# YoungSean/UnseenObjectsWithMeanShift

Measured on AMD Instinct MI355X. Metric: images/sec @640x480 RGB-D, 100 queries, 9 decoder layers; % MFMA roofline, higher is better.
Workload: dtype f32; 1 GPU; configs[1]: batch 8 of 640x480 per GPU, ResNet-50 features -> MSDeformAttn pixel decoder -> 9-layer decoder, 100 q ->~; global_batch=8, per_gpu_batch=8, launch=hipgraph x4: 4 batches of 8 in flight, one graph + stream each, batches_in_flight=4, parallelism=dp1, GPU_MAX_HW_QUEUES=4, visible_gpus=1, rank0_numa=pinned

## Files before the change

### include/msm_hip.h

```cpp
#ifndef MSM_HIP_H
#define MSM_HIP_H

#include <stdint.h>

#ifdef __cplusplus
extern "C" {
#endif

#define MSM_OK 0
#define MSM_E_INVALID (-1)
#define MSM_E_LAUNCH (-2)
#define MSM_E_WORKSPACE (-3)

const char* msm_last_error_string(void);
#define MSM_ABI_VERSION 24
int msm_abi_version(void);

#define MSM_OPT_AUTO (-1)
enum {
    MSM_OPT_MASK_NC = 0,
    MSM_OPT_MASKB_TARGET,
    MSM_OPT_GEMM_TILE,
    MSM_OPT_GEMM_SHALLOW,
    MSM_OPT_ATTN_TARGET,
    MSM_OPT_ATTN_KERNEL,
    MSM_OPT_ATTN_QK_MAX,
    MSM_OPT_ATTN_QKCFG,
    MSM_OPT_CONVIN_NT,
    MSM_OPT_POST_GENERIC,
    MSM_OPT_ENC_NO_COOP,
    MSM_OPT_MSDA_GENERIC,
    MSM_OPT_MS_CHUNK,
    MSM_OPT_MS_NO_PERSISTENT,
    MSM_OPT_ATTN_FUSED_KV,
    MSM_OPT_KV_PIPE,
    MSM_OPT_MASK_KERNEL,
    MSM_OPT_MS_SPLIT_KERNEL,
    MSM_OPT_CONV3_WIDE,
    MSM_OPT_DEC_TILE32,
    MSM_OPT_COUNT
};
int msm_set_option(int key, int value);
int msm_get_option(int key);

int msm_gemm_f32(const float* A, const float* A2, const float* W, const float* bias, float* C,
                 int M, int N, int K, int batch,
                 int64_t a_sm, int64_t a_sk, int64_t a_sb, int64_t a2_sb, int64_t w_sb,
                 int64_t c_sm, int64_t c_sn, int64_t c_sb, int64_t c_ss,
                 int a_mode, int conv_h, int conv_w, int conv_c,
                 int bias_mode, int act, int split_k, void* stream);

int msm_layernorm_f32(const float* x, const float* parts, int n_parts, int64_t part_stride,
                      const float* bias, const float* g1, const float* b1, int l2norm,
                      const float* g2, const float* b2, float* y, float* y2,
                      int rows, int E, float eps, void* stream);

int msm_groupnorm_stats_f32(const float* x, double* stats, int stats_cleared, int B, int HW, int C, void* stream);
int msm_groupnorm_apply_f32(const float* x, const double* stats, const float* gamma, const float* beta,
                            const float* up, int uh, int uw, int64_t up_batch_stride, float* y,
                            int B, int H, int W, int C, int groups, float eps, int relu, void* stream);

int msm_groupnorm_apply_split(const float* x, const double* stats, const float* gamma, const float* beta,
                              const float* up, int uh, int uw, int64_t up_batch_stride, uint16_t* planes,
                              int B, int H, int W, int C, int groups, float eps, int relu, void* stream);

int msm_groupnorm_apply_f16(const float* x, const double* stats, const float* gamma, const float* beta,
                            const float* up, int uh, int uw, int64_t up_batch_stride, void* y_f16,
                            int B, int H, int W, int C, int groups, float eps, int relu, void* stream);
// ... 34 lines not shown
int64_t msm_hypersphere_attn_workspace(int B, int Lq, int S, int heads);
int msm_hypersphere_attn_fwd(const float* q, const float* k, const float* v,
                             const uint8_t* masked, const int32_t* row_any, float* out,
                             int B, int Lq, int S, int heads,
                             int64_t ldq, int64_t q_sb, int64_t ldk, int64_t k_sb,
                             int64_t ldv, int64_t v_sb, float kappa,
                             float* workspace, int64_t workspace_elems, void* stream);
int msm_hypersphere_attn_lp_fwd(const float* q, const void* k, const void* v, int kv_format,
                                const uint8_t* masked, const int32_t* row_any, float* out,
                                int B, int Lq, int S, int heads,
                                int64_t ldq, int64_t q_sb, int64_t ldk, int64_t k_sb,
                                int64_t ldv, int64_t v_sb, float kappa,
                                float* workspace, int64_t workspace_elems, void* stream);

int msm_nchw_to_tokens_f16(const float* in, void* out, int B, int C, int HW, void* stream);
int msm_attn_pack_kv_weights(const float* w, void* packed, int heads, void* stream);
int msm_mask_conv3x3_folded(const void* x_f16, const float* F, int64_t ldf, int64_t f_sb, void* mask_bits, int32_t* row_any, int row_any_cleared,
                            float* logits, int B, int Q, int H, int W, void* stream);
int64_t msm_attn_mask_bits_bytes(int B, int Lq, int S);
int msm_attn_pack_mask_bits(const uint8_t* masked, void* bits, int B, int Lq, int S, void* stream);
int msm_hypersphere_attn_fused_kv_fwd(const float* q, const void* x_f16, const void* w_packed, const float* rowcol, const float* col_v_t,
                                      int score_format, const void* mask_bits, const int32_t* row_any, float* out,
                                      int B, int Lq, int H, int W, int heads, int64_t ldq, int64_t q_sb, float kappa,
                                      float* workspace, int64_t workspace_elems, void* stream);

int msm_msdeform_attn_fwd(const float* value, const int64_t* spatial_shapes,
                          const int64_t* level_start_index, const float* sampling_loc,
                          const float* attn_weight, float* out,
                          int B, int S, int M, int D, int L, int Lq, int P, void* stream);

int msm_msdeform_attn_bwd(const float* value, const int64_t* spatial_shapes,
                          const int64_t* level_start_index, const float* sampling_loc,
                          const float* attn_weight, const float* grad_output,
                          float* grad_value, float* grad_sampling_loc, float* grad_attn_weight,
                          int B, int S, int M, int D, int L, int Lq, int P, void* stream);
int msm_msdeform_attn_fwd_f64(const double* value, const int64_t* spatial_shapes,
                              const int64_t* level_start_index, const double* sampling_loc,
                              const double* attn_weight, double* out,
                              int B, int S, int M, int D, int L, int Lq, int P, void* stream);
int msm_msdeform_attn_bwd_f64(const double* value, const int64_t* spatial_shapes,
                              const int64_t* level_start_index, const double* sampling_loc,
                              const double* attn_weight, const double* grad_output,
                              double* grad_value, double* grad_sampling_loc, double* grad_attn_weight,
                              int B, int S, int M, int D, int L, int Lq, int P, void* stream);

int msm_msdeform_attn_enc_fwd(const float* value, const int64_t* spatial_shapes,
                              const int64_t* level_start_index, const float* proj, float* out,
                              int B, int S, int M, int D, int L, int P, void* stream);

int msm_value_to_head_major_f32(const float* value, float* value_hm, int B, int S, int M, int D, void* stream);
int msm_msdeform_attn_enc_hm_fwd(const float* value_hm, const int64_t* spatial_shapes,
                                 const int64_t* level_start_index, const float* proj, float* out,
                                 int B, int S, int M, int D, int L, int P, void* stream);

int msm_msda_pack_proj(const float* w , const float* bias, float* wpack, float* bpack,
                       int M, int L, int P, void* stream);
int msm_msdeform_attn_enc_fused_fwd(const float* value_hm, const int64_t* spatial_shapes, const int64_t* level_start_index,
                                    const float* src, const float* pos, const float* wpack, const float* bpack, float* out,
                                    int B, int S, int M, int D, int L, int P, void* stream);

int64_t msm_encoder_block_stream_floats(int d_ffn, int proj_width);
int msm_encoder_block_fwd(const float* attn, const float* src, const float* wstream, const float* small,
                          const float* pos, float* src_out, float* value_out, float* proj_out,
                          int M, int S, int d_ffn, int proj_width, int value_heads, float eps, void* stream);

int msm_kv_project_f32(const float* x, const float* w, const float* cmat, float* out,
                       int B, int C, int HW, int N, int x_tokens, int64_t x_batch_stride, int cmat_width, void* stream);
int msm_kv_project_multi_f32(int n_jobs, const float* const* x, const float* const* w, const float* const* cmat,
                             float* const* out, const int32_t* HW, const int32_t* x_tokens, const int64_t* x_batch_stride,
                             const int32_t* cmat_width, int B, int C, int N, void* stream);
int msm_kv_project_multi_bf16(int n_jobs, const float* const* x, const float* const* w, const float* const* cmat,
                              uint16_t* const* out, const int32_t* HW, const int32_t* x_tokens, const int64_t* x_batch_stride,
                              const int32_t* cmat_width, int B, int C, int N, int half_format, void* stream);
int msm_kv_project_multi_split(int n_jobs, const float* const* x, const float* const* w, const float* const* cmat,
                               float* const* out, const int32_t* HW, const int32_t* x_tokens, const int64_t* x_batch_stride,
                               const int32_t* cmat_width, int B, int C, int N, void* stream);

int msm_tokens_proj_nchw_f32(const float* x, const float* w, const float* bias, const double* gn_stats,
                             const float* gn_gamma, const float* gn_beta, int groups, float eps, int relu, float* out,
                             int B, int C, int HW, int N, void* stream);

int msm_dec_pack_weight(const float* w, float* packed, int N, int K, void* stream);
int msm_dec_post_cross(const float* attn_out, const float* res, const float* query_pos,
                       const float* wo, const float* bo, const float* ln_g, const float* ln_b,
                       const float* w_in, const float* b_in,
                       float* x_out, float* qk_out, float* v_out,
                       int rows, int Q, int E, float eps, void* stream);
int msm_dec_post_self(const float* attn_out, const float* res,
                      const float* wo, const float* bo, const float* ln_g, const float* ln_b,
                      const float* w1, const float* b1, const float* w2, int F,
                      float* x_out, float* parts, int n_parts, int rows, int E, float eps, void* stream);
int msm_dec_heads(const float* x, const float* parts, int n_parts, const float* bias,
                  const float* ln_g, const float* ln_b, int l2norm,
                  const float* dec_g, const float* dec_b,
                  const float* m0w, const float* m0b, const float* m1w, const float* m1b,
                  const float* m2w, const float* m2b,
                  const float* wq, const float* bq, const float* query_pos,
                  float* out, float* d_out, float* e_out, float* q_out, int32_t* row_any_zero,
                  int rows, int Q, int E, float eps, void* stream);

int msm_dec_pack_weight_bf16(const float* w, uint16_t* packed, int N, int K, void* stream);
int msm_dec_post_cross_bf16(const float* attn_out, const float* res, const float* query_pos,
                            const uint16_t* wo, const float* bo, const float* ln_g, const float* ln_b,
                            const uint16_t* w_in, const float* b_in,
                            float* x_out, float* qk_out, float* v_out,
                            int rows, int Q, int E, float eps, void* stream);
// ... 213 lines not shown
```

### unseenobjectswithmeanshift_amd/_lib.py

```python
import ctypes
import os
import re

_HERE = os.path.dirname(os.path.abspath(__file__))
LIB_PATH = os.path.join(_HERE, "libmsm_hip.so")
HEADER_PATH = os.path.join(os.path.dirname(_HERE), "include", "msm_hip.h")

_lib = None
ABI_VERSION = 24

c_f = ctypes.c_void_p
c_p = ctypes.c_void_p
c_i = ctypes.c_int
c_l = ctypes.c_int64
c_fl = ctypes.c_float

_SIGNATURES = {
    "msm_abi_version": (c_i, []),
    "msm_last_error_string": (ctypes.c_char_p, []),
    "msm_set_option": (c_i, [c_i, c_i]),
    "msm_get_option": (c_i, [c_i]),
    "msm_gemm_f32": (c_i, [c_f, c_f, c_f, c_f, c_f, c_i, c_i, c_i, c_i,
                           c_l, c_l, c_l, c_l, c_l, c_l, c_l, c_l, c_l,
                           c_i, c_i, c_i, c_i, c_i, c_i, c_i, c_p]),
    "msm_layernorm_f32": (c_i, [c_f, c_f, c_i, c_l, c_f, c_f, c_f, c_i, c_f, c_f, c_f, c_f, c_i, c_i, c_fl, c_p]),
    "msm_groupnorm_stats_f32": (c_i, [c_f, c_p, c_i, c_i, c_i, c_i, c_p]),
    "msm_groupnorm_apply_f32": (c_i, [c_f, c_p, c_f, c_f, c_f, c_i, c_i, c_l, c_f, c_i, c_i, c_i, c_i, c_i, c_fl, c_i, c_p]),
    "msm_groupnorm_apply_split": (c_i, [c_f, c_p, c_f, c_f, c_f, c_i, c_i, c_l, c_f, c_i, c_i, c_i, c_i, c_i, c_fl, c_i, c_p]),
    "msm_groupnorm_apply_f16": (c_i, [c_f, c_p, c_f, c_f, c_f, c_i, c_i, c_l, c_p, c_i, c_i, c_i, c_i, c_i, c_fl, c_i, c_p]),
    "msm_groupnorm_apply_nchw_f32": (c_i, [c_f, c_p, c_f, c_f, c_f, c_i, c_i, c_i, c_i, c_fl, c_i, c_p]),
    "msm_pos_embed_sine": (c_i, [c_f, c_i, c_i, c_i, c_l, c_l, c_f, c_fl, c_fl, c_p]),
    "msm_transpose_f32": (c_i, [c_f, c_f, c_i, c_i, c_i, c_p]),
    "msm_l2_normalize_nchw_f32": (c_i, [c_f, c_f, c_i, c_i, c_i, c_fl, c_p]),
    "msm_msda_locations": (c_i, [c_f, c_f, c_f, c_p, c_f, c_f, c_l, c_i, c_i, c_i, c_p]),
    "msm_mask_logits_fwd": (c_i, [c_f, c_f, c_f, c_p, c_p, c_i, c_i, c_i, c_i, c_i, c_i, c_i, c_i, c_l, c_f, c_l, c_p]),
    "msm_pool_mask_taps": (c_i, [c_f, c_i, c_i, c_i, c_i, c_p, c_p, c_p, c_p, c_l, c_p]),
    "msm_attn_mask_pooled": (c_i, [c_f, c_l, c_f, c_l, c_f, c_p, c_p, c_i, c_i, c_i, c_i, c_i, c_p]),
    "msm_pack_mask_features_bf16": (c_i, [c_f, c_p, c_i, c_i, c_i, c_p]),
    "msm_pack_mask_features_f16": (c_i, [c_f, c_p, c_i, c_i, c_i, c_p]),
    "msm_mask_logits_bf16_fwd": (c_i, [c_f, c_p, c_f, c_p, c_p, c_i, c_i, c_i, c_i, c_i, c_i, c_i, c_i, c_l, c_f, c_l, c_p]),
    "msm_pack_mask_features_split": (c_i, [c_f, c_p, c_i, c_i, c_i, c_p]),
    "msm_mask_logits_split_fwd": (c_i, [c_f, c_p, c_f, c_p, c_p, c_i, c_i, c_i, c_i, c_i, c_i, c_i, c_i, c_l, c_f, c_l, c_p]),
    "msm_hypersphere_attn_workspace": (c_l, [c_i, c_i, c_i, c_i]),
    "msm_hypersphere_attn_fwd": (c_i, [c_f, c_f, c_f, c_p, c_p, c_f, c_i, c_i, c_i, c_i,
                                       c_l, c_l, c_l, c_l, c_l, c_l, c_fl, c_f, c_l, c_p]),
    "msm_hypersphere_attn_lp_fwd": (c_i, [c_f, c_p, c_p, c_i, c_p, c_p, c_f, c_i, c_i, c_i, c_i,
                                          c_l, c_l, c_l, c_l, c_l, c_l, c_fl, c_f, c_l, c_p]),
    "msm_hypersphere_attn_bwd_workspace": (c_l, [c_i, c_i, c_i]),
    "msm_hypersphere_attn_bwd": (c_i, [c_f, c_f, c_f, c_p, c_p, c_f, c_f, c_f, c_f, c_i, c_i, c_i, c_i,
                                       c_l, c_l, c_l, c_l, c_l, c_l, c_fl, c_f, c_l, c_p]),
    "msm_msdeform_attn_fwd": (c_i, [c_f, c_p, c_p, c_f, c_f, c_f, c_i, c_i, c_i, c_i, c_i, c_i, c_i, c_p]),
    "msm_msdeform_attn_bwd": (c_i, [c_f, c_p, c_p, c_f, c_f, c_f, c_f, c_f, c_f, c_i, c_i, c_i, c_i, c_i, c_i, c_i, c_p]),
    "msm_msdeform_attn_fwd_f64": (c_i, [c_f, c_p, c_p, c_f, c_f, c_f, c_i, c_i, c_i, c_i, c_i, c_i, c_i, c_p]),
    "msm_msdeform_attn_bwd_f64": (c_i, [c_f, c_p, c_p, c_f, c_f, c_f, c_f, c_f, c_f, c_i, c_i, c_i, c_i, c_i, c_i, c_i, c_p]),
    "msm_msdeform_attn_enc_fwd": (c_i, [c_f, c_p, c_p, c_f, c_f, c_i, c_i, c_i, c_i, c_i, c_i, c_p]),
    "msm_encoder_block_stream_floats": (c_l, [c_i, c_i]),
    "msm_value_to_head_major_f32": (c_i, [c_f, c_f, c_i, c_i, c_i, c_i, c_p]),
    "msm_msdeform_attn_enc_hm_fwd": (c_i, [c_f, c_p, c_p, c_f, c_f, c_i, c_i, c_i, c_i, c_i, c_i, c_p]),
    "msm_msda_pack_proj": (c_i, [c_f, c_f, c_f, c_f, c_i, c_i, c_i, c_p]),
    "msm_msdeform_attn_enc_fused_fwd": (c_i, [c_f, c_p, c_p, c_f, c_f, c_f, c_f, c_f, c_i, c_i, c_i, c_i, c_i, c_i, c_p]),
    "msm_encoder_block_fwd": (c_i, [c_f, c_f, c_f, c_f, c_f, c_f, c_f, c_f, c_i, c_i, c_i, c_i, c_i, c_fl, c_p]),
    "msm_encoder_block_split_stream_bytes": (c_l, [c_i, c_i]),
    "msm_encoder_block_split_fwd": (c_i, [c_f, c_f, c_p, c_f, c_f, c_f, c_f, c_f, c_i, c_i, c_i, c_i, c_i, c_fl, c_p]),
    "msm_encoder_block_lp_stream_bytes": (c_l, [c_i, c_i]),
    "msm_encoder_block_lp_fwd": (c_i, [c_f, c_f, c_p, c_f, c_f, c_f, c_f, c_f, c_i, c_i, c_i, c_i, c_i, c_fl, c_p]),
    "msm_encoder_block_hm_stream_bytes": (c_l, [c_i, c_i]),
    "msm_encoder_block_hm_small_floats": (c_i, [c_i]),
    "msm_encoder_block_hm_fwd": (c_i, [c_p, c_f, c_p, c_f, c_f, c_f, c_p, c_p, c_i, c_i, c_i, c_fl, c_i, c_p]),
    "msm_msdeform_attn_enc_lp_fwd": (c_i, [c_p, c_p, c_p, c_p, c_p, c_i, c_i, c_i, c_i, c_i, c_i, c_p]),
    "msm_msdeform_attn_enc_lp_fused_fwd": (c_i, [c_p, c_p, c_p, c_f, c_f, c_p, c_f, c_p, c_i, c_i, c_i, c_i, c_i, c_i, c_p]),
    "msm_f32_to_f16": (c_i, [c_f, c_p, c_l, c_p]),
    "msm_bias_act_nhwc": (c_i, [c_p, c_p, c_p, c_i, c_l, c_i, c_i, c_p]),
    "msm_nhwc_to_nchw_f32": (c_i, [c_p, c_f, c_i, c_i, c_i, c_i, c_p]),
    "msm_ucn_embedding_tail": (c_i, [c_f, c_f, c_f, c_i, c_i, c_i, c_i, c_i, c_i, c_fl, c_p]),
    "msm_f32_to_f16_rows": (c_i, [c_f, c_p, c_i, c_l, c_l, c_p]),
    "msm_kv_project_f32": (c_i, [c_f, c_f, c_f, c_f, c_i, c_i, c_i, c_i, c_i, c_l, c_i, c_p]),
    "msm_kv_project_multi_f32": (c_i, [c_i, c_p, c_p, c_p, c_p, c_p, c_p, c_p, c_p, c_i, c_i, c_i, c_p]),
    "msm_kv_project_multi_bf16": (c_i, [c_i, c_p, c_p, c_p, c_p, c_p, c_p, c_p, c_p, c_i, c_i, c_i, c_i, c_p]),
    "msm_kv_project_multi_split": (c_i, [c_i, c_p, c_p, c_p, c_p, c_p, c_p, c_p, c_p, c_i, c_i, c_i, c_p]),
    "msm_tokens_proj_nchw_f32": (c_i, [c_f, c_f, c_f, c_p, c_f, c_f, c_i, c_fl, c_i, c_f, c_i, c_i, c_i, c_i, c_p]),
    "msm_dec_pack_weight": (c_i, [c_f, c_f, c_i, c_i, c_p]),
    "msm_dec_post_cross": (c_i, [c_f] * 12 + [c_i, c_i, c_i, c_fl, c_p]),
    "msm_dec_post_self": (c_i, [c_f] * 9 + [c_i, c_f, c_f, c_i, c_i, c_i, c_fl, c_p]),
    "msm_dec_heads": (c_i, [c_f, c_f, c_i, c_f, c_f, c_f, c_i] + [c_f] * 15 + [c_p, c_i, c_i, c_i, c_fl, c_p]),
    "msm_dec_pack_weight_bf16": (c_i, [c_f, c_p, c_i, c_i, c_p]),
    "msm_dec_post_cross_bf16": (c_i, [c_f, c_f, c_f, c_p, c_f, c_f, c_f, c_p, c_f, c_f, c_f, c_f] + [c_i, c_i, c_i, c_fl, c_p]),
    "msm_dec_post_self_bf16": (c_i, [c_f, c_f, c_p, c_f, c_f, c_f, c_p, c_f, c_p] + [c_i, c_f, c_f, c_i, c_i, c_i, c_fl, c_p]),
    "msm_dec_heads_bf16": (c_i, [c_f, c_f, c_i, c_f, c_f, c_f, c_i, c_f, c_f, c_p, c_f, c_p, c_f, c_p, c_f, c_p, c_f, c_f] + [c_f] * 4 +
                           [c_p, c_i, c_i, c_i, c_fl, c_p]),
    "msm_nchw_to_tokens_f16": (c_i, [c_f, c_p, c_i, c_i, c_i, c_p]),
    "msm_mask_conv3x3_folded": (c_i, [c_p, c_f, c_l, c_l, c_p, c_p, c_i, c_f, c_i, c_i, c_i, c_i, c_p]),
    "msm_attn_pack_kv_weights": (c_i, [c_f, c_p, c_i, c_p]),
    "msm_attn_mask_bits_bytes": (c_l, [c_i, c_i, c_i]),
    "msm_attn_pack_mask_bits": (c_i, [c_p, c_p, c_i, c_i, c_i, c_p]),
    "msm_hypersphere_attn_fused_kv_fwd": (c_i, [c_f, c_p, c_p, c_f, c_f, c_i, c_p, c_p, c_f, c_i, c_i, c_i, c_i, c_i, c_l, c_l, c_fl, c_f, c_l, c_p]),
    "msm_dec_pack_weight_f16": (c_i, [c_f, c_p, c_i, c_i, c_p]),
    "msm_dec_post_cross_f16": (c_i, [c_f, c_f, c_f, c_p, c_f, c_f, c_f, c_p, c_f, c_f, c_f, c_f] + [c_i, c_i, c_i, c_fl, c_p]),
    "msm_dec_post_self_f16": (c_i, [c_f, c_f, c_p, c_f, c_f, c_f, c_p, c_f, c_p] + [c_i, c_f, c_f, c_i, c_i, c_i, c_fl, c_p]),
    "msm_dec_heads_f16": (c_i, [c_f, c_f, c_i, c_f, c_f, c_f, c_i, c_f, c_f, c_p, c_f, c_p, c_f, c_p, c_f, c_p, c_f, c_f] + [c_f] * 4 +
                          [c_p, c_i, c_i, c_i, c_fl, c_p]),
    "msm_dec_heads_mask": (c_i, [c_f, c_f, c_i, c_f, c_f, c_f, c_i, c_f, c_f, c_p, c_f, c_p, c_f, c_p, c_f, c_p, c_f, c_f] + [c_f] * 4 +
                           [c_f, c_i, c_i, c_p, c_p, c_i, c_i, c_i, c_i, c_fl, c_p]),
    "msm_dec_pack_weight_bf16x2": (c_i, [c_f, c_p, c_i, c_i, c_p]),
    "msm_dec_post_cross_bf16x2": (c_i, [c_f, c_f, c_f, c_p, c_f, c_f, c_f, c_p, c_f, c_f, c_f, c_f] + [c_i, c_i, c_i, c_fl, c_p]),
    "msm_dec_post_self_bf16x2": (c_i, [c_f, c_f, c_p, c_f, c_f, c_f, c_p, c_f, c_p] + [c_i, c_f, c_f, c_i, c_i, c_i, c_fl, c_p]),
    "msm_dec_heads_bf16x2": (c_i, [c_f, c_f, c_i, c_f, c_f, c_f, c_i, c_f, c_f, c_p, c_f, c_p, c_f, c_p, c_f, c_p, c_f, c_f] + [c_f] * 4 +
                             [c_p, c_i, c_i, c_i, c_fl, c_p]),
    "msm_l2_prefetch": (c_i, [c_p, c_p, c_i, c_p]),
    "msm_dec_set_prefetch": (c_i, [c_p, c_p, c_i]),
    "msm_ms_seed_workspace": (c_l, [c_i]),
    "msm_ms_select_seeds": (c_i, [c_f, c_i, c_i, c_i, c_l, c_f, c_p, c_f, c_l, c_i, c_p]),
# ... 148 lines not shown
```

### unseenobjectswithmeanshift_amd/csrc/msda.hip

```cpp
#include <stdlib.h>

#include "common.h"

namespace msm {

constexpr int MAXL = 8;

template <int V>
struct Vec {
    float e[V];
};
template <int V>
__device__ __forceinline__ Vec<V> ldv(const float* p) {
    Vec<V> r;
    if constexpr (V == 4) {
        const float4 t = *reinterpret_cast<const float4*>(p);
        r.e[0] = t.x; r.e[1] = t.y; r.e[2] = t.z; r.e[3] = t.w;
    } else {
#pragma unroll
        for (int i = 0; i < V; ++i) r.e[i] = p[i];
    }
    return r;
}

// ... 322 lines not shown
                const int i = i0 + j;
                wt[j] = wb[j] = 0.f;
                vt[j] = vbm[j] = make_float4(0.f, 0.f, 0.f, 0.f);
                if (i < LP) {
                    int W = Ws[0], H = Hs[0], s0 = 0;
#pragma unroll
                    for (int l = 1; l < MAXL; ++l)
                        if (l < L && i >= l * P) { W = Ws[l]; H = Hs[l]; s0 = st[l]; }
                    const float w_im = quad_bcast(px[i >> 2], i & 3);
                    const float h_im = quad_bcast(py[i >> 2], i & 3);
                    const float wgt = quad_bcast(pw[i >> 2], i & 3) * rden;
                    const float hf = floorf(h_im), wf = floorf(w_im);
                    const int h_low = (int)hf, xw = (int)wf + cx;
                    const float lh = h_im - hf, lw = w_im - wf;
                    const float wxw = (unsigned)xw < (unsigned)W ? (cx ? lw : 1.f - lw) * wgt : 0.f;
                    wt[j] = (unsigned)h_low < (unsigned)H ? (1.f - lh) * wxw : 0.f;
                    wb[j] = (unsigned)(h_low + 1) < (unsigned)H ? lh * wxw : 0.f;
                    const int xc = clamp0(xw, W - 1);
                    const int yt = clamp0(h_low, H - 1), yb = clamp0(h_low + 1, H - 1);
                    const unsigned col = vlane + (unsigned)(s0 + xc) * (unsigned)(D * 4);
                    vt[j] = ldv4(vrsrc, col + __umul24((unsigned)yt, (unsigned)(W * D * 4)));
                    vbm[j] = ldv4(vrsrc, col + __umul24((unsigned)yb, (unsigned)(W * D * 4)));
                }
            }
#pragma unroll
            for (int j = 0; j < GP; ++j) {
                acc.x += wt[j] * vt[j].x + wb[j] * vbm[j].x;
                acc.y += wt[j] * vt[j].y + wb[j] * vbm[j].y;
                acc.z += wt[j] * vt[j].z + wb[j] * vbm[j].z;
                acc.w += wt[j] * vt[j].w + wb[j] * vbm[j].w;
            }
        }
    }
    acc.x += __int_as_float(__builtin_amdgcn_mov_dpp(__float_as_int(acc.x), 0x4E, 0xf, 0xf, true));
    acc.y += __int_as_float(__builtin_amdgcn_mov_dpp(__float_as_int(acc.y), 0x4E, 0xf, 0xf, true));
    acc.z += __int_as_float(__builtin_amdgcn_mov_dpp(__float_as_int(acc.z), 0x4E, 0xf, 0xf, true));
    acc.w += __int_as_float(__builtin_amdgcn_mov_dpp(__float_as_int(acc.w), 0x4E, 0xf, 0xf, true));
    if (live && cx == 0) *reinterpret_cast<float4*>(out + (((int64_t)b * S + qi) * M + m) * D + d4 * 4) = acc;
}

struct LevelRcp {
    float rw[4], rh[4];
};
__device__ __forceinline__ float div_by(float x, float W, float rW) {
    const float q = x * rW;
    return fmaf(fmaf(-q, W, x), rW, q);
}
__device__ __forceinline__ float exp_neg(float x) { return __builtin_amdgcn_exp2f(x * 1.4426950408889634f); }
__device__ __forceinline__ float rcp_nr(float x) {
    const float r = __builtin_amdgcn_rcpf(x);
    return fmaf(fmaf(-x, r, 1.0f), r, r);
}

template <int LC, int PC>
__global__ __launch_bounds__(256) void msda_enc_hm8_rec_kernel(const float* __restrict__ value, const int64_t* __restrict__ shapes,
                                                               const int64_t* __restrict__ lstart, const float* __restrict__ proj,
                                                               float* __restrict__ out, int B, int S, int M) {
    constexpr int D = 8, LP = LC * PC, SLOTS = LP / 4;
    static_assert(PC == 4 && LP % 4 == 0 && LP <= 16, "a lane owns one point of every level: PC == 4");
    constexpr int QSTRIDE = LP * 2 + 1;
    __shared__ float4 recs[4 * 16 * QSTRIDE];
    const int b = blockIdx.x % B;
    const int blk = blockIdx.x / B;
    const int tid = threadIdx.x, lane = tid & 63;
    const int wave = __builtin_amdgcn_readfirstlane(tid >> 6);
    const int g = tid & 3, cx = g >> 1, d4 = g & 1;
    const int m = blk % M;
    const int q_raw = (blk / M) * 64 + (tid >> 2);
    const bool live = q_raw < S;
    const int qi = live ? q_raw : 0;

    int Hs[LC], Ws[LC], st[LC];
#pragma unroll
    for (int l = 0; l < LC; ++l) {
        Hs[l] = (int)shapes[2 * l];
        Ws[l] = (int)shapes[2 * l + 1];
        st[l] = (int)lstart[l];
    }
    LevelRcp lr;
#pragma unroll
    for (int l = 0; l < LC; ++l) {
        lr.rw[l] = rcp_nr((float)Ws[l]);
        lr.rh[l] = rcp_nr((float)Hs[l]);
    }
    const float* pr = proj + ((int64_t)b * S + qi) * (M * LP * 3);
    const float* offp = pr + (int64_t)m * LP * 2;
    const float* lgp = pr + (int64_t)M * LP * 2 + (int64_t)m * LP;
    int qW = Ws[0], qH = Hs[0], qs = 0;
    float qrw = lr.rw[0], qrh = lr.rh[0];
#pragma unroll
    for (int l = 1; l < LC; ++l)
        if (qi >= st[l]) { qW = Ws[l]; qH = Hs[l]; qs = st[l]; qrw = lr.rw[l]; qrh = lr.rh[l]; }
    const int local = qi - qs;
    const int ry = (int)(((float)local + 0.5f) * qrw), rx = local - ry * qW;
    const float ref_x = div_by((float)rx + 0.5f, (float)qW, qrw);
    const float ref_y = div_by((float)ry + 0.5f, (float)qH, qrh);

    float px[SLOTS], py[SLOTS], pw[SLOTS];
    float mx = -INFINITY;
#pragma unroll
    for (int slot = 0; slot < SLOTS; ++slot) {
        const int i = slot * 4 + g;
        const float2 off = *reinterpret_cast<const float2*>(offp + 2 * i);
        const float lg = lgp[i];
        const float lx = ref_x + div_by(off.x, (float)Ws[slot], lr.rw[slot]);
        const float ly = ref_y + div_by(off.y, (float)Hs[slot], lr.rh[slot]);
        px[slot] = lx * (float)Ws[slot] - 0.5f;
        py[slot] = ly * (float)Hs[slot] - 0.5f;
        pw[slot] = lg;
        mx = fmaxf(mx, lg);
    }
    mx = quad_max(mx);
    float den = 0.f;
#pragma unroll
    for (int slot = 0; slot < SLOTS; ++slot) {
        pw[slot] = exp_neg(pw[slot] - mx);
        den += pw[slot];
    }
    const float rden = rcp_nr(quad_sum(den));

    float4* qrec = recs + (wave * 16 + (lane >> 2)) * QSTRIDE;
#pragma unroll
    for (int slot = 0; slot < SLOTS; ++slot) {
        const int W = Ws[slot], H = Hs[slot], s0 = st[slot];
        const float w_im = px[slot], h_im = py[slot];
        const float wgt = pw[slot] * rden;
        const float hf = floorf(h_im), wf = floorf(w_im);
        const int h_low = (int)hf, w_low = (int)wf;
        const float lh = h_im - hf, lw = w_im - wf;
        const float wx0 = (unsigned)w_low < (unsigned)W ? (1.f - lw) * wgt : 0.f;
        const float wx1 = (unsigned)(w_low + 1) < (unsigned)W ? lw * wgt : 0.f;
        const bool okt = (unsigned)h_low < (unsigned)H, okb = (unsigned)(h_low + 1) < (unsigned)H;
        const unsigned rowt = __umul24((unsigned)clamp0(h_low, H - 1), (unsigned)(W * D * 4));
        const unsigned rowb = __umul24((unsigned)clamp0(h_low + 1, H - 1), (unsigned)(W * D * 4));
        const unsigned c0 = (unsigned)(s0 + clamp0(w_low, W - 1)) * (unsigned)(D * 4);
        const unsigned c1 = (unsigned)(s0 + clamp0(w_low + 1, W - 1)) * (unsigned)(D * 4);
        const int i = slot * 4 + g;
        qrec[i * 2 + 0] = make_float4(__uint_as_float(c0 + rowt), __uint_as_float(c0 + rowb), okt ? (1.f - lh) * wx0 : 0.f, okb ? lh * wx0 : 0.f);
        qrec[i * 2 + 1] = make_float4(__uint_as_float(c1 + rowt), __uint_as_float(c1 + rowb), okt ? (1.f - lh) * wx1 : 0.f, okb ? lh * wx1 : 0.f);
    }
    __builtin_amdgcn_fence(__ATOMIC_RELEASE, "wavefront");
    __builtin_amdgcn_wave_barrier();
    __builtin_amdgcn_fence(__ATOMIC_ACQUIRE, "wavefront");

    const uint64_t vbase = (uint64_t)(value + ((int64_t)b * M + m) * S * D);
    const __amdgpu_buffer_rsrc_t vrsrc = __builtin_amdgcn_make_buffer_rsrc(
        (void*)(((uint64_t)(unsigned)__builtin_amdgcn_readfirstlane((int)(vbase >> 32)) << 32) | (uint64_t)(unsigned)__builtin_amdgcn_readfirstlane((int)(unsigned)vbase)),
        0, S * D * 4, 0x00020000);
    const unsigned lane_off = (unsigned)d4 * 16u;
    const float4* myrec = qrec + cx;
    float4 acc = make_float4(0.f, 0.f, 0.f, 0.f);
    constexpr int GP = 4;
#pragma unroll
    for (int i0 = 0; i0 < LP; i0 += GP) {
        float4 vt[GP], vbm[GP], r[GP];
#pragma unroll
        for (int j = 0; j < GP; ++j) {
            r[j] = myrec[(i0 + j) * 2];
            vt[j] = ldv4(vrsrc, __float_as_uint(r[j].x) + lane_off);
            vbm[j] = ldv4(vrsrc, __float_as_uint(r[j].y) + lane_off);
        }
#pragma unroll
        for (int j = 0; j < GP; ++j) {
            acc.x += r[j].z * vt[j].x + r[j].w * vbm[j].x;
            acc.y += r[j].z * vt[j].y + r[j].w * vbm[j].y;
            acc.z += r[j].z * vt[j].z + r[j].w * vbm[j].z;
            acc.w += r[j].z * vt[j].w + r[j].w * vbm[j].w;
        }
    }
    acc.x += __int_as_float(__builtin_amdgcn_mov_dpp(__float_as_int(acc.x), 0x4E, 0xf, 0xf, true));
    acc.y += __int_as_float(__builtin_amdgcn_mov_dpp(__float_as_int(acc.y), 0x4E, 0xf, 0xf, true));
    acc.z += __int_as_float(__builtin_amdgcn_mov_dpp(__float_as_int(acc.z), 0x4E, 0xf, 0xf, true));
    acc.w += __int_as_float(__builtin_amdgcn_mov_dpp(__float_as_int(acc.w), 0x4E, 0xf, 0xf, true));
    if (live && cx == 0) *reinterpret_cast<float4*>(out + (((int64_t)b * S + qi) * M + m) * D + d4 * 4) = acc;
}

template <int LC, int PC>
__global__ __launch_bounds__(256) void msda_enc_hm8_fused_kernel(const float* __restrict__ value, const int64_t* __restrict__ shapes,
                                                                 const int64_t* __restrict__ lstart, const float* __restrict__ src,
                                                                 const float* __restrict__ pos, const float4* __restrict__ wpack,
                                                                 const float* __restrict__ bpack, float* __restrict__ out, int B,
                                                                 int S, int M) {
    constexpr int D = 8, LP = LC * PC, SLOTS = LP / 4, EC = 64;
    static_assert(PC == 4 && LP == 12, "three 16-row blocks hold the 36 projection rows of a head");
    constexpr int QSTRIDE = LP * 2 + 1;
    constexpr int TSTRIDE = 52;
    constexpr int WF4 = 3 * 4 * 64;
    static_assert(WF4 + 4 * 16 * TSTRIDE / 4 == 4 * 16 * QSTRIDE, "phase-A layout fills the record region exactly");
    __shared__ float4 recs[4 * 16 * QSTRIDE];
    const int b = blockIdx.x % B;
    const int blk = blockIdx.x / B;
    const int tid = threadIdx.x, lane = tid & 63;
    const int wave = __builtin_amdgcn_readfirstlane(tid >> 6);
    const int m = blk % M;
    const int q0 = (blk / M) * 64 + wave * 16;

    const int lj = lane & 15, lq = lane >> 4;
    float x[4][4];
    {
        const int tk = min(q0 + lj, S - 1);
        float4 a[4], p[4];
#pragma unroll
        for (int fb = 0; fb < 4; ++fb) {
            a[fb] = *reinterpret_cast<const float4*>(src + ((int64_t)b * S + tk) * EC + fb * 16 + lq * 4);
            p[fb] = *reinterpret_cast<const float4*>(pos + (int64_t)tk * EC + fb * 16 + lq * 4);
        }
#pragma unroll
        for (int i = 0; i < WF4 / 256; ++i) recs[i * 256 + tid] = wpack[m * WF4 + i * 256 + tid];
#pragma unroll
        for (int fb = 0; fb < 4; ++fb) {
            x[fb][0] = a[fb].x + p[fb].x; x[fb][1] = a[fb].y + p[fb].y; x[fb][2] = a[fb].z + p[fb].z; x[fb][3] = a[fb].w + p[fb].w;
        }
    }
    int Hs[LC], Ws[LC], st[LC];
#pragma unroll
    for (int l = 0; l < LC; ++l) {
        Hs[l] = (int)shapes[2 * l];
        Ws[l] = (int)shapes[2 * l + 1];
        st[l] = (int)lstart[l];
    }
    LevelRcp lr;
#pragma unroll
    for (int l = 0; l < LC; ++l) {
        lr.rw[l] = rcp_nr((float)Ws[l]);
        lr.rh[l] = rcp_nr((float)Hs[l]);
    }
    __syncthreads();
// ... 279 lines not shown
    MSM_REQUIRE(value && spatial_shapes && level_start_index && proj && out, "msm_msdeform_attn_enc_fwd: null pointer");
    int rc = msda_common_checks("msm_msdeform_attn_enc_fwd", value, out, B, S, M, D, L, S, P);
    if (rc != MSM_OK) return rc;
    const int V = (D % 4 == 0) ? 4 : 1;
    const int64_t per_img = (int64_t)S * M * (D / V);
    dim3 grid((unsigned)(((per_img + 255) / 256) * B)), block(256);
    if (V == 4)
        hipLaunchKernelGGL((msda_kernel<true, 4>), grid, block, 0, (hipStream_t)stream, value, spatial_shapes,
                           level_start_index, (const float*)nullptr, (const float*)nullptr, proj, out, B, S, M, D, L, S, P);
    else
        hipLaunchKernelGGL((msda_kernel<true, 1>), grid, block, 0, (hipStream_t)stream, value, spatial_shapes,
                           level_start_index, (const float*)nullptr, (const float*)nullptr, proj, out, B, S, M, D, L, S, P);
    MSM_CHECK_LAUNCH("msm_msdeform_attn_enc_fwd");
    return MSM_OK;
}

extern "C" int msm_msdeform_attn_bwd(const float* value, const int64_t* spatial_shapes, const int64_t* level_start_index,
                                     const float* sampling_loc, const float* attn_weight, const float* grad_output,
                                     float* grad_value, float* grad_sampling_loc, float* grad_attn_weight, int B, int S,
                                     int M, int D, int L, int Lq, int P, void* stream) {
    MSM_REQUIRE(value && spatial_shapes && level_start_index && sampling_loc && attn_weight && grad_output && grad_value &&
                    grad_sampling_loc && grad_attn_weight,
                "msm_msdeform_attn_bwd: null pointer");
    if (D > 64 || L > MAXL)
        return msda_any_bwd_f32(value, spatial_shapes, level_start_index, sampling_loc, attn_weight, grad_output, grad_value,
                                grad_sampling_loc, grad_attn_weight, B, S, M, D, L, Lq, P, stream);
    int rc = msda_common_checks("msm_msdeform_attn_bwd", value, grad_output, B, S, M, D, L, Lq, P);
    if (rc != MSM_OK) return rc;
    MSM_REQUIRE((((uintptr_t)grad_value) & 15) == 0, "msm_msdeform_attn_bwd: grad_value must be 16-byte aligned");
    hipStream_t st = (hipStream_t)stream;
    const int V = (D % 4 == 0) ? 4 : 1;
    const int D4 = D / V;
    const bool pow2 = (D4 & (D4 - 1)) == 0;
    MSM_CHECK_HIP(hipMemsetAsync(grad_value, 0, sizeof(float) * (size_t)B * S * M * D, st));
    if (!pow2) {
        MSM_CHECK_HIP(hipMemsetAsync(grad_sampling_loc, 0, sizeof(float) * (size_t)B * Lq * M * L * P * 2, st));
        MSM_CHECK_HIP(hipMemsetAsync(grad_attn_weight, 0, sizeof(float) * (size_t)B * Lq * M * L * P, st));
    }
    const int64_t per_img = (int64_t)Lq * M * D4;
    dim3 grid((unsigned)(((per_img + 255) / 256) * B)), block(256);
#define MSDA_BWD(VV, PP)                                                                                              \
    hipLaunchKernelGGL((msda_bwd_kernel<VV, PP>), grid, block, 0, st, value, spatial_shapes, level_start_index,        \
                       sampling_loc, attn_weight, grad_output, grad_value, grad_sampling_loc, grad_attn_weight, B, S, M, \
                       D, L, Lq, P)
    if (V == 4 && pow2) MSDA_BWD(4, true);
    else if (V == 4) MSDA_BWD(4, false);
    else if (pow2) MSDA_BWD(1, true);
    else MSDA_BWD(1, false);
#undef MSDA_BWD
    MSM_CHECK_LAUNCH("msm_msdeform_attn_bwd");
    return MSM_OK;
}

extern "C" int msm_msdeform_attn_enc_hm_fwd(const float* value_hm, const int64_t* spatial_shapes,
                                            const int64_t* level_start_index, const float* proj, float* out, int B, int S,
                                            int M, int D, int L, int P, void* stream) {
    MSM_REQUIRE(value_hm && spatial_shapes && level_start_index && proj && out, "msm_msdeform_attn_enc_hm_fwd: null pointer");
    int rc = msda_common_checks("msm_msdeform_attn_enc_hm_fwd", value_hm, out, B, S, M, D, L, S, P);
    if (rc != MSM_OK) return rc;
    const int V = (D % 4 == 0) ? 4 : 1;
    const int G = 2 * (D / V);
    MSM_REQUIRE(256 % G == 0, "msm_msdeform_attn_enc_hm_fwd: D=%d: 2*D/%d lanes per head must divide 256", D, V);
    MSM_REQUIRE((int64_t)S * D < ((int64_t)1 << 31), "msm_msdeform_attn_enc_hm_fwd: S*D must fit 31 bits");
    const int64_t per_img = (int64_t)S * M * G;
    dim3 grid((unsigned)(((per_img + 255) / 256) * B)), block(256);
    if (D == 8 && L * P <= 16 && (int64_t)M * S * D * 4 < ((int64_t)1 << 31) && opt(MSM_OPT_MSDA_GENERIC) == 3)
        hipLaunchKernelGGL((msda_enc_hm8_kernel<false, 0, 0>), grid, block, 0, (hipStream_t)stream, value_hm, spatial_shapes,
                           level_start_index, proj, out, B, S, M, L, P);
    else if (D == 8 && L == 3 && P == 4 && (int64_t)S * D * 4 < ((int64_t)1 << 31) && opt(MSM_OPT_MSDA_GENERIC) == MSM_OPT_AUTO)
        hipLaunchKernelGGL((msda_enc_hm8_rec_kernel<3, 4>), dim3((unsigned)(cdiv(S, 64) * M * B)), block, 0, (hipStream_t)stream, value_hm,
                           spatial_shapes, level_start_index, proj, out, B, S, M);
    else if (D == 8 && L == 3 && P == 4 && (int64_t)M * S * D * 4 < ((int64_t)1 << 31) && opt(MSM_OPT_MSDA_GENERIC) != 1)
        hipLaunchKernelGGL((msda_enc_hm8_kernel<true, 3, 4>), dim3((unsigned)(cdiv(S, 64) * M * B)), block, 0, (hipStream_t)stream, value_hm,
                           spatial_shapes, level_start_index, proj, out, B, S, M, L, P);
    else if (D == 8 && L * P <= 16 && (int64_t)M * S * D * 4 < ((int64_t)1 << 31) && opt(MSM_OPT_MSDA_GENERIC) != 1)
        hipLaunchKernelGGL((msda_enc_hm8_kernel<true, 0, 0>), dim3((unsigned)(cdiv(S, 64) * M * B)), block, 0, (hipStream_t)stream, value_hm,
                           spatial_shapes, level_start_index, proj, out, B, S, M, L, P);
    else if (V == 4)
        hipLaunchKernelGGL((msda_enc_hm_kernel<4>), grid, block, 0, (hipStream_t)stream, value_hm, spatial_shapes,
                           level_start_index, proj, out, B, S, M, D, L, P);
    else
        hipLaunchKernelGGL((msda_enc_hm_kernel<1>), grid, block, 0, (hipStream_t)stream, value_hm, spatial_shapes,
                           level_start_index, proj, out, B, S, M, D, L, P);
    MSM_CHECK_LAUNCH("msm_msdeform_attn_enc_hm_fwd");
    return MSM_OK;
}

extern "C" int msm_msda_pack_proj(const float* w, const float* bias, float* wpack, float* bpack, int M, int L, int P, void* stream) {
    MSM_REQUIRE(w && bias && wpack && bpack, "msm_msda_pack_proj: null pointer");
    MSM_REQUIRE(M > 0 && L * P == 12, "msm_msda_pack_proj: L*P=%d, the fused gather takes 12 sampling points per head", L * P);
    MSM_REQUIRE(((((uintptr_t)w) | ((uintptr_t)wpack)) & 15) == 0, "msm_msda_pack_proj: pointers must be 16-byte aligned");
    hipLaunchKernelGGL(msda_pack_proj_kernel, dim3((unsigned)cdiv(M * 768, 256)), dim3(256), 0, (hipStream_t)stream, w, bias,
                       reinterpret_cast<float4*>(wpack), bpack, M, L * P);
    MSM_CHECK_LAUNCH("msm_msda_pack_proj");
    return MSM_OK;
}

extern "C" int msm_msdeform_attn_enc_fused_fwd(const float* value_hm, const int64_t* spatial_shapes, const int64_t* level_start_index,
                                               const float* src, const float* pos, const float* wpack, const float* bpack, float* out,
                                               int B, int S, int M, int D, int L, int P, void* stream) {
    MSM_REQUIRE(value_hm && spatial_shapes && level_start_index && src && pos && wpack && bpack && out,
                "msm_msdeform_attn_enc_fused_fwd: null pointer");
    MSM_REQUIRE(B > 0 && S > 0 && M > 0, "msm_msdeform_attn_enc_fused_fwd: bad sizes");
    MSM_REQUIRE(D == 8 && M * D == 64 && L == 3 && P == 4,
                "msm_msdeform_attn_enc_fused_fwd: only the pixel decoder's geometry (64 channels = 8 heads x 8, 3 levels x 4 points); got M=%d D=%d L=%d P=%d",
                M, D, L, P);
    MSM_REQUIRE((int64_t)S * D * 4 < ((int64_t)1 << 31), "msm_msdeform_attn_enc_fused_fwd: S too large");
    MSM_REQUIRE(((((uintptr_t)value_hm) | ((uintptr_t)src) | ((uintptr_t)pos) | ((uintptr_t)wpack) | ((uintptr_t)bpack) | ((uintptr_t)out)) & 15) == 0,
                "msm_msdeform_attn_enc_fused_fwd: pointers must be 16-byte aligned");
    hipLaunchKernelGGL((msda_enc_hm8_fused_kernel<3, 4>), dim3((unsigned)(cdiv(S, 64) * M * B)), dim3(256), 0, (hipStream_t)stream, value_hm,
                       spatial_shapes, level_start_index, src, pos, reinterpret_cast<const float4*>(wpack), bpack, out, B, S, M);
    MSM_CHECK_LAUNCH("msm_msdeform_attn_enc_fused_fwd");
    return MSM_OK;
}

extern "C" int msm_value_to_head_major_f32(const float* value, float* value_hm, int B, int S, int M, int D, void* stream) {
    MSM_REQUIRE(value && value_hm && value != value_hm, "msm_value_to_head_major_f32: null or aliased pointer");
    MSM_REQUIRE(B > 0 && S > 0 && M > 0 && D > 0 && D % 4 == 0, "msm_value_to_head_major_f32: D=%d must be a multiple of 4", D);
    MSM_REQUIRE(((((uintptr_t)value) | ((uintptr_t)value_hm)) & 15) == 0, "msm_value_to_head_major_f32: pointers must be 16-byte aligned");
    const int64_t total4 = (int64_t)B * S * M * (D / 4);
    hipLaunchKernelGGL(value_to_hm_kernel, dim3((unsigned)min((int64_t)2048, (total4 + 255) / 256)), dim3(256), 0,
                       (hipStream_t)stream, value, value_hm, total4, S, M, D / 4);
// ... 4 lines not shown
```

Baseline: 3791 images/sec.

## Add persistent MSDA encoder kernel with prefetched projection loads

Splits the record-based MSDA encoder kernel into geometry, projection-load, record-build and gather helpers, and loads projections through buffer resource descriptors. It adds a persistent variant that loops over work units and prefetches the next unit's projection while gathering the current one, plus an occupancy hint on the default kernel (launch_bounds 256,6). The persistent path is only taken when the MSDA_GENERIC option is set between 11 and 18, so by default only the buffer-load rewrite and the occupancy bound apply. Compile-time probe macros can replace loads with synthetic values to isolate costs.

```diff
diff --git a/include/msm_hip.h b/include/msm_hip.h
--- a/include/msm_hip.h
+++ b/include/msm_hip.h
@@ -13,7 +13,7 @@
 #define MSM_E_WORKSPACE (-3)
 
 const char* msm_last_error_string(void);
-#define MSM_ABI_VERSION 24
+#define MSM_ABI_VERSION 25
 int msm_abi_version(void);
 
 #define MSM_OPT_AUTO (-1)
@@ -154,6 +154,7 @@
 int msm_msdeform_attn_enc_hm_fwd(const float* value_hm, const int64_t* spatial_shapes,
                                  const int64_t* level_start_index, const float* proj, float* out,
                                  int B, int S, int M, int D, int L, int P, void* stream);
+int msm_msda_persist_workgroups(int B);
 
 int msm_msda_pack_proj(const float* w , const float* bias, float* wpack, float* bpack,
                        int M, int L, int P, void* stream);
diff --git a/unseenobjectswithmeanshift_amd/_lib.py b/unseenobjectswithmeanshift_amd/_lib.py
--- a/unseenobjectswithmeanshift_amd/_lib.py
+++ b/unseenobjectswithmeanshift_amd/_lib.py
@@ -7,7 +7,7 @@
 HEADER_PATH = os.path.join(os.path.dirname(_HERE), "include", "msm_hip.h")
 
 _lib = None
-ABI_VERSION = 24
+ABI_VERSION = 25
 
 c_f = ctypes.c_void_p
 c_p = ctypes.c_void_p
@@ -57,6 +57,7 @@
     "msm_encoder_block_stream_floats": (c_l, [c_i, c_i]),
     "msm_value_to_head_major_f32": (c_i, [c_f, c_f, c_i, c_i, c_i, c_i, c_p]),
     "msm_msdeform_attn_enc_hm_fwd": (c_i, [c_f, c_p, c_p, c_f, c_f, c_i, c_i, c_i, c_i, c_i, c_i, c_p]),
+    "msm_msda_persist_workgroups": (c_i, [c_i]),
     "msm_msda_pack_proj": (c_i, [c_f, c_f, c_f, c_f, c_i, c_i, c_i, c_p]),
     "msm_msdeform_attn_enc_fused_fwd": (c_i, [c_f, c_p, c_p, c_f, c_f, c_f, c_f, c_f, c_i, c_i, c_i, c_i, c_i, c_i, c_p]),
     "msm_encoder_block_fwd": (c_i, [c_f, c_f, c_f, c_f, c_f, c_f, c_f, c_f, c_i, c_i, c_i, c_i, c_i, c_fl, c_p]),
diff --git a/unseenobjectswithmeanshift_amd/csrc/msda.hip b/unseenobjectswithmeanshift_amd/csrc/msda.hip
--- a/unseenobjectswithmeanshift_amd/csrc/msda.hip
+++ b/unseenobjectswithmeanshift_amd/csrc/msda.hip
@@ -398,40 +398,72 @@
     return fmaf(fmaf(-x, r, 1.0f), r, r);
 }
 
+
+#ifndef MSDA_REC_PARTS
+#define MSDA_REC_PARTS 0
+#endif
+template <int LC>
+struct RecGeom {
+    int Hs[LC], Ws[LC], st[LC];
+    LevelRcp lr;
+};
+template <int LC>
+__device__ __forceinline__ RecGeom<LC> rec_geometry(const int64_t* __restrict__ shapes, const int64_t* __restrict__ lstart) {
+    RecGeom<LC> ge;
+#pragma unroll
+    for (int l = 0; l < LC; ++l) {
+        ge.Hs[l] = (int)shapes[2 * l];
+        ge.Ws[l] = (int)shapes[2 * l + 1];
+        ge.st[l] = (int)lstart[l];
+    }
+#pragma unroll
+    for (int l = 0; l < LC; ++l) {
+        ge.lr.rw[l] = rcp_nr((float)ge.Ws[l]);
+        ge.lr.rh[l] = rcp_nr((float)ge.Hs[l]);
+    }
+    return ge;
+}
+template <int SLOTS>
+struct RecProj {
+    float2 off[SLOTS];
+    float lg[SLOTS];
+};
+__device__ __forceinline__ __amdgpu_buffer_rsrc_t rec_proj_rsrc(const float* __restrict__ proj, int b, int S, int M, int LP) {
+    const uint64_t pbase = (uint64_t)(proj + (int64_t)b * S * (M * LP * 3));
+    return __builtin_amdgcn_make_buffer_rsrc(
+        (void*)(((uint64_t)(unsigned)__builtin_amdgcn_readfirstlane((int)(pbase >> 32)) << 32) | (uint64_t)(unsigned)__builtin_amdgcn_readfirstlane((int)(unsigned)pbase)),
+        0, S * M * LP * 3 * 4, 0x00020000);
+}
+typedef unsigned int msda_u32x2 __attribute__((ext_vector_type(2)));
+template <int SLOTS>
+__device__ __forceinline__ RecProj<SLOTS> rec_load_proj(__amdgpu_buffer_rsrc_t prsrc, int M, int m, int qi, int g) {
+    constexpr int LP = SLOTS * 4;
+    const unsigned row = (unsigned)qi * (unsigned)(M * LP * 3);
+    const unsigned offw = row + (unsigned)(m * LP * 2 + 2 * g);
+    const unsigned lgw = row + (unsigned)(M * LP * 2 + m * LP + g);
+    RecProj<SLOTS> pj;
+#pragma unroll
+    for (int slot = 0; slot < SLOTS; ++slot) {
+#if MSDA_REC_PARTS & 1
+        const int i = slot * 4 + g;
+        pj.off[slot] = make_float2((float)((qi + i) & 7) - 3.5f, (float)((qi >> 3) & 7) - 3.5f);
+        pj.lg[slot] = (float)((qi + m + i) & 15) * 0.125f;
+        asm volatile("" ::"v"(offw), "v"(lgw), "s"(prsrc));
+#else
+        const msda_u32x2 o = __builtin_amdgcn_raw_buffer_load_b64(prsrc, (offw + 8 * slot) * 4u, 0, 0);
+        pj.off[slot] = make_float2(__uint_as_float(o.x), __uint_as_float(o.y));
+        pj.lg[slot] = __uint_as_float(__builtin_amdgcn_raw_buffer_load_b32(prsrc, (lgw + 4 * slot) * 4u, 0, 0));
+#endif
+    }
+    return pj;
+}
 template <int LC, int PC>
-__global__ __launch_bounds__(256) void msda_enc_hm8_rec_kernel(const float* __restrict__ value, const int64_t* __restrict__ shapes,
-                                                               const int64_t* __restrict__ lstart, const float* __restrict__ proj,
-                                                               float* __restrict__ out, int B, int S, int M) {
+__device__ __forceinline__ void rec_records(const RecGeom<LC>& ge, const RecProj<LC * PC / 4>& pj, float4* __restrict__ qrec, int qi, int g) {
     constexpr int D = 8, LP = LC * PC, SLOTS = LP / 4;
-    static_assert(PC == 4 && LP % 4 == 0 && LP <= 16, "a lane owns one point of every level: PC == 4");
-    constexpr int QSTRIDE = LP * 2 + 1;
-    __shared__ float4 recs[4 * 16 * QSTRIDE];
-    const int b = blockIdx.x % B;
-    const int blk = blockIdx.x / B;
-    const int tid = threadIdx.x, lane = tid & 63;
-    const int wave = __builtin_amdgcn_readfirstlane(tid >> 6);
-    const int g = tid & 3, cx = g >> 1, d4 = g & 1;
-    const int m = blk % M;
-    const int q_raw = (blk / M) * 64 + (tid >> 2);
-    const bool live = q_raw < S;
-    const int qi = live ? q_raw : 0;
-
-    int Hs[LC], Ws[LC], st[LC];
-#pragma unroll
-    for (int l = 0; l < LC; ++l) {
-        Hs[l] = (int)shapes[2 * l];
-        Ws[l] = (int)shapes[2 * l + 1];
-        st[l] = (int)lstart[l];
-    }
-    LevelRcp lr;
-#pragma unroll
-    for (int l = 0; l < LC; ++l) {
-        lr.rw[l] = rcp_nr((float)Ws[l]);
-        lr.rh[l] = rcp_nr((float)Hs[l]);
-    }
-    const float* pr = proj + ((int64_t)b * S + qi) * (M * LP * 3);
-    const float* offp = pr + (int64_t)m * LP * 2;
-    const float* lgp = pr + (int64_t)M * LP * 2 + (int64_t)m * LP;
+    const int* Hs = ge.Hs;
+    const int* Ws = ge.Ws;
+    const int* st = ge.st;
+    const LevelRcp& lr = ge.lr;
     int qW = Ws[0], qH = Hs[0], qs = 0;
     float qrw = lr.rw[0], qrh = lr.rh[0];
 #pragma unroll
@@ -446,9 +478,8 @@
     float mx = -INFINITY;
 #pragma unroll
     for (int slot = 0; slot < SLOTS; ++slot) {
-        const int i = slot * 4 + g;
-        const float2 off = *reinterpret_cast<const float2*>(offp + 2 * i);
-        const float lg = lgp[i];
+        const float2 off = pj.off[slot];
+        const float lg = pj.lg[slot];
         const float lx = ref_x + div_by(off.x, (float)Ws[slot], lr.rw[slot]);
         const float ly = ref_y + div_by(off.y, (float)Hs[slot], lr.rh[slot]);
         px[slot] = lx * (float)Ws[slot] - 0.5f;
@@ -465,7 +496,6 @@
     }
     const float rden = rcp_nr(quad_sum(den));
 
-    float4* qrec = recs + (wave * 16 + (lane >> 2)) * QSTRIDE;
 #pragma unroll
     for (int slot = 0; slot < SLOTS; ++slot) {
         const int W = Ws[slot], H = Hs[slot], s0 = st[slot];
@@ -488,7 +518,12 @@
     __builtin_amdgcn_fence(__ATOMIC_RELEASE, "wavefront");
     __builtin_amdgcn_wave_barrier();
     __builtin_amdgcn_fence(__ATOMIC_ACQUIRE, "wavefront");
-
+}
+template <int LC, int PC>
+__device__ __forceinline__ void rec_gather(const float4* __restrict__ qrec, const float* __restrict__ value, float* __restrict__ out, int b,
+                                           int S, int M, int m, int qi, bool live, int g) {
+    constexpr int D = 8, LP = LC * PC;
+    const int cx = g >> 1, d4 = g & 1;
     const uint64_t vbase = (uint64_t)(value + ((int64_t)b * M + m) * S * D);
     const __amdgpu_buffer_rsrc_t vrsrc = __builtin_amdgcn_make_buffer_rsrc(
         (void*)(((uint64_t)(unsigned)__builtin_amdgcn_readfirstlane((int)(vbase >> 32)) << 32) | (uint64_t)(unsigned)__builtin_amdgcn_readfirstlane((int)(unsigned)vbase)),
@@ -503,8 +538,14 @@
 #pragma unroll
         for (int j = 0; j < GP; ++j) {
             r[j] = myrec[(i0 + j) * 2];
+#if MSDA_REC_PARTS & 2
+            asm volatile("" ::"v"(__float_as_uint(r[j].x) + lane_off), "v"(__float_as_uint(r[j].y) + lane_off), "s"(vrsrc));
+            vt[j] = make_float4(r[j].z, r[j].w, r[j].z, r[j].w);
+            vbm[j] = make_float4(r[j].w, r[j].z, r[j].w, r[j].z);
+#else
             vt[j] = ldv4(vrsrc, __float_as_uint(r[j].x) + lane_off);
             vbm[j] = ldv4(vrsrc, __float_as_uint(r[j].y) + lane_off);
+#endif
         }
 #pragma unroll
         for (int j = 0; j < GP; ++j) {
@@ -519,6 +560,73 @@
     acc.z += __int_as_float(__builtin_amdgcn_mov_dpp(__float_as_int(acc.z), 0x4E, 0xf, 0xf, true));
     acc.w += __int_as_float(__builtin_amdgcn_mov_dpp(__float_as_int(acc.w), 0x4E, 0xf, 0xf, true));
     if (live && cx == 0) *reinterpret_cast<float4*>(out + (((int64_t)b * S + qi) * M + m) * D + d4 * 4) = acc;
+}
+
+template <int LC, int PC>
+__global__ __launch_bounds__(256, 6) void msda_enc_hm8_rec_kernel(const float* __restrict__ value, const int64_t* __restrict__ shapes,
+                                                               const int64_t* __restrict__ lstart, const float* __restrict__ proj,
+                                                               float* __restrict__ out, int B, int S, int M) {
+    constexpr int LP = LC * PC, SLOTS = LP / 4;
+    static_assert(PC == 4 && LP % 4 == 0 && LP <= 16, "a lane owns one point of every level: PC == 4");
+    constexpr int QSTRIDE = LP * 2 + 1;
+    __shared__ float4 recs[4 * 16 * QSTRIDE];
+    const int b = blockIdx.x % B;
+    const int blk = blockIdx.x / B;
+    const int tid = threadIdx.x, lane = tid & 63;
+    const int wave = __builtin_amdgcn_readfirstlane(tid >> 6);
+    const int g = tid & 3;
+    const int m = blk % M;
+    const int q_raw = (blk / M) * 64 + (tid >> 2);
+    const bool live = q_raw < S;
+    const int qi = live ? q_raw : 0;
+    const RecGeom<LC> ge = rec_geometry<LC>(shapes, lstart);
+    const RecProj<SLOTS> pj = rec_load_proj<SLOTS>(rec_proj_rsrc(proj, b, S, M, LP), M, m, qi, g);
+    float4* qrec = recs + (wave * 16 + (lane >> 2)) * QSTRIDE;
+    rec_records<LC, PC>(ge, pj, qrec, qi, g);
+    rec_gather<LC, PC>(qrec, value, out, b, S, M, m, qi, live, g);
+}
+
+#ifndef MSDA_PERSIST_WAVES
+#define MSDA_PERSIST_WAVES 5
+#endif
+template <int LC, int PC>
+__global__ __launch_bounds__(256, MSDA_PERSIST_WAVES) void msda_enc_hm8_rec_persist_kernel(const float* __restrict__ value, const int64_t* __restrict__ shapes,
+                                                                       const int64_t* __restrict__ lstart, const float* __restrict__ proj,
+                                                                       float* __restrict__ out, int B, int S, int M) {
+    constexpr int LP = LC * PC, SLOTS = LP / 4;
+    static_assert(PC == 4 && LP % 4 == 0 && LP <= 16, "a lane owns one point of every level: PC == 4");
+    constexpr int QSTRIDE = LP * 2 + 1;
+    __shared__ float4 recs[4 * 16 * QSTRIDE];
+    const int b = blockIdx.x % B;
+    const int first = blockIdx.x / B;
+    const int nwg = ((int)gridDim.x - b + B - 1) / B;
+    const int units = ((S + 63) >> 6) * M;
+    if (first >= units) return;
+    const int tid = threadIdx.x, lane = tid & 63;
+    const int wave = __builtin_amdgcn_readfirstlane(tid >> 6);
+    const int g = tid & 3;
+    float4* qrec = recs + (wave * 16 + (lane >> 2)) * QSTRIDE;
+    const RecGeom<LC> ge = rec_geometry<LC>(shapes, lstart);
+    const int dq = nwg / M, dm = nwg - dq * M;
+    int qb = first / M, m = first - qb * M;
+    int q_raw = qb * 64 + (tid >> 2);
+    const __amdgpu_buffer_rsrc_t prsrc = rec_proj_rsrc(proj, b, S, M, LP);
+    RecProj<SLOTS> pj = rec_load_proj<SLOTS>(prsrc, M, m, q_raw < S ? q_raw : 0, g);
+    for (int u = first; u < units; u += nwg) {
+        const bool live = q_raw < S;
+        const int qi = live ? q_raw : 0;
+        int qb_n = qb + dq, m_n = m + dm;
+        if (m_n >= M) { m_n -= M; ++qb_n; }
+        if (u + nwg >= units) { qb_n = qb; m_n = m; }
+        const int q_raw_n = qb_n * 64 + (tid >> 2);
+        rec_records<LC, PC>(ge, pj, qrec, qi, g);
+        pj = rec_load_proj<SLOTS>(prsrc, M, m_n, q_raw_n < S ? q_raw_n : 0, g);
+        __builtin_amdgcn_sched_barrier(0x38f);
+        rec_gather<LC, PC>(qrec, value, out, b, S, M, m, qi, live, g);
+        __builtin_amdgcn_fence(__ATOMIC_RELEASE, "wavefront");
+        __builtin_amdgcn_wave_barrier();
+        qb = qb_n; m = m_n; q_raw = q_raw_n;
+    }
 }
 
 template <int LC, int PC>
@@ -904,6 +1012,22 @@
     return MSM_OK;
 }
 
+static int msda_persist_grid(int B) {
+    static int cus[64];
+    const int o = opt(MSM_OPT_MSDA_GENERIC);
+    if (!(o > 10 && o <= 18)) return 0;
+    int dev = 0, n = 0;
+    if (hipGetDevice(&dev) != hipSuccess || dev < 0 || dev >= 64) return 0;
+    if (cus[dev] <= 0) {
+        if (hipDeviceGetAttribute(&n, hipDeviceAttributeMultiprocessorCount, dev) != hipSuccess || n <= 0) n = 256;
+        cus[dev] = n;
+    }
+    const int grid = cus[dev] * (o - 10);
+    return grid >= B ? grid : 0;
+}
+
+extern "C" int msm_msda_persist_workgroups(int B) { return B > 0 ? msda_persist_grid(B) : 0; }
+
 extern "C" int msm_msdeform_attn_enc_hm_fwd(const float* value_hm, const int64_t* spatial_shapes,
                                             const int64_t* level_start_index, const float* proj, float* out, int B, int S,
                                             int M, int D, int L, int P, void* stream) {
@@ -916,10 +1040,15 @@
     MSM_REQUIRE((int64_t)S * D < ((int64_t)1 << 31), "msm_msdeform_attn_enc_hm_fwd: S*D must fit 31 bits");
     const int64_t per_img = (int64_t)S * M * G;
     dim3 grid((unsigned)(((per_img + 255) / 256) * B)), block(256);
+    const bool rec_proj_fits = (int64_t)S * M * L * P * 3 * 4 < ((int64_t)1 << 31);
     if (D == 8 && L * P <= 16 && (int64_t)M * S * D * 4 < ((int64_t)1 << 31) && opt(MSM_OPT_MSDA_GENERIC) == 3)
         hipLaunchKernelGGL((msda_enc_hm8_kernel<false, 0, 0>), grid, block, 0, (hipStream_t)stream, value_hm, spatial_shapes,
                            level_start_index, proj, out, B, S, M, L, P);
-    else if (D == 8 && L == 3 && P == 4 && (int64_t)S * D * 4 < ((int64_t)1 << 31) && opt(MSM_OPT_MSDA_GENERIC) == MSM_OPT_AUTO)
+    else if (D == 8 && L == 3 && P == 4 && (int64_t)S * D * 4 < ((int64_t)1 << 31) && rec_proj_fits && msda_persist_grid(B) > 0)
+        hipLaunchKernelGGL((msda_enc_hm8_rec_persist_kernel<3, 4>), dim3((unsigned)msda_persist_grid(B)), block, 0, (hipStream_t)stream,
+                           value_hm, spatial_shapes, level_start_index, proj, out, B, S, M);
+    else if (D == 8 && L == 3 && P == 4 && (int64_t)S * D * 4 < ((int64_t)1 << 31) && rec_proj_fits &&
+             (opt(MSM_OPT_MSDA_GENERIC) == MSM_OPT_AUTO || opt(MSM_OPT_MSDA_GENERIC) == 4 || opt(MSM_OPT_MSDA_GENERIC) > 10))
         hipLaunchKernelGGL((msda_enc_hm8_rec_kernel<3, 4>), dim3((unsigned)(cdiv(S, 64) * M * B)), block, 0, (hipStream_t)stream, value_hm,
                            spatial_shapes, level_start_index, proj, out, B, S, M);
     else if (D == 8 && L == 3 && P == 4 && (int64_t)M * S * D * 4 < ((int64_t)1 << 31) && opt(MSM_OPT_MSDA_GENERIC) != 1)
```

Result: no change. 3800 images/sec (median of 6 runs) (+0.2%).
